# RViMLab/MICCAI2021_Cataract_semantic_segmentation

Hardware: AMD Instinct MI355X
Metric: train frames/sec @540x960 OCRNet-HRNetw48 (higher is better)
Workload: dtype f32 (convolutions with K >= 2048 and >= 192 output columns, and the 3x3 trunk convolutions of the HRNet widths: forward / backward-data of those with > 192 output columns: operands scaled by a per-tensor power of two and split into 2 fp16 planes (22 significant bits), 3 fp16 MFMA products; forward /

## Files before the change

### include/catseg_debug.h

```cpp
#ifndef CATSEG_DEBUG_H
#define CATSEG_DEBUG_H

#include "catseg.h"

#ifdef __cplusplus
extern "C" {
#endif

int catseg_debug_set_tile(int mi, int ni);
int catseg_debug_set_splits(int splits);
int catseg_debug_set_strided_multi(int on);
int catseg_debug_set_lovasz_prune(int on);
int catseg_debug_set_wgrad_direct(int on);

int catseg_debug_set_dconv3_blocks(int blocks);
int catseg_debug_set_dconv3_spec(int on);
int catseg_debug_set_dconv3_alt96(int on);
int catseg_debug_set_dwgrad3_blocks(int blocks);
int catseg_debug_set_dwgrad3_pl_blocks(int blocks);
int catseg_debug_set_dwgrad3_pl_form(int form);
int catseg_debug_set_dconv3_pl_slots(int slots);
int catseg_debug_set_dconv3_pl_pair(int mask);
int catseg_debug_dconv3_pl_occupancy(int C, int pair);
int catseg_debug_dwgrad3_pl_occupancy(int C);

int catseg_debug_set_h2w_slow_epilogue(int on);

int catseg_debug_set_b3_tile(int t);
int catseg_debug_plan_conv(const catseg_conv_desc* d, int op, int* out);

int catseg_debug_set_bilinear_bwd_fused(int on);
int catseg_debug_set_h2w_waves(int waves);

int catseg_debug_set_pconv1_wgrad_blocks(int n);

#ifdef __cplusplus
}
#endif
#endif
```

### miccai2021_cataract_semantic_segmentation_amd/_lib.py

```python
import ctypes as C
import os

import torch

_HERE = os.path.dirname(os.path.abspath(__file__))
LIB_PATH = os.environ.get("CATSEG_LIB") or os.path.join(_HERE, "libcatseg_hip.so")

if not os.path.exists(LIB_PATH):
    raise ImportError(
        "libcatseg_hip.so is missing (%s). Build it with `python -c 'import __graft_entry__ as g; g.build()'` "
        "or `make -C miccai2021_cataract_semantic_segmentation_amd/csrc`. There is no CPU fallback." % LIB_PATH)

lib = C.CDLL(LIB_PATH)

P, I, L, F, SZ = C.c_void_p, C.c_int, C.c_longlong, C.c_float, C.c_size_t


class ConvDesc(C.Structure):
    _fields_ = [(n, I) for n in ("B", "H", "W", "Cin", "Ho", "Wo", "Cout", "kh", "kw", "stride", "pad", "dil",
                                 "ldx", "ldy", "stem4", "groups")]


class BnApplyDesc(C.Structure):
    _fields_ = [("y", P), ("ldy", I), ("mean", P), ("scale", P), ("beta", P), ("residual", P), ("ldr", I), ("residual_record", P), ("z", P), ("ldz", I),
# ... 36 lines not shown
    "catseg_dconv3_pl_rows": (I, [I, I, I, I]),
    "catseg_planes_bytes": (SZ, [L, I]),
    "catseg_planes_from_f32": (I, [P, I, L, I, P, P, I, P]),
    "catseg_dconv3_pl": (I, [I, I, I, I, P, P, P, P, P, P, I, I, P, SZ, P, P, P]),
    "catseg_dconv3_pl_bnbwd": (I, [I, I, I, I, P, P, P, P, P, I, P, I, P, P, P, P, SZ, P, P]),
    "catseg_dwgrad3_pl_supported": (I, [I]),
    "catseg_dwgrad3_pl_workspace": (SZ, [I, I, I, I]),
    "catseg_dwgrad3_pl": (I, [I, I, I, I, P, P, P, P, P, P, SZ, P]),
    "catseg_bn_finalize_counts_bound": (I, [P, I, P, L, I, P, P, F, F, P, P, P, P, P, P, P]),
    "catseg_bn_backward_h2_workspace": (SZ, [L, I]),
    "catseg_head_fwd": (I, [P, I, P, P, P, P, P, I, L, I, P, I, I, P]),
    "catseg_head_backward_workspace": (SZ, [L, I]),
    "catseg_head_backward": (I, [P, I, P, I, P, P, P, P, I, L, I, P, P, P, P, P, P, P, P, P, P, P, SZ, P]),
    "catseg_head_fwd_drop": (I, [P, I, P, P, P, P, P, I, L, I, P, I, I, P, L, F, P]),
    "catseg_head_backward_drop": (I, [P, I, P, I, P, P, P, P, I, L, I, P, P, P, P, P, P, P, P, P, P, P, SZ, P, L, F, P]),
    "catseg_dropout2d_mask": (I, [P, F, I, I, P, P, P]),
    "catseg_dropout2d_mask_fixed": (I, [P, F, I, I, P, P, P]),
    "catseg_dropout2d_apply": (I, [P, I, P, L, I, L, P, I, P]),
    "catseg_maxpool2x2_fwd": (I, [P, I, P, I, P, I, I, I, I, P]),
    "catseg_maxpool2x2_bwd": (I, [P, I, P, P, I, I, I, I, I, P]),
    "catseg_bias_rows": (I, [P, P, I, L, I, P]),
    "catseg_bn_mask_bytes": (SZ, [L, I]),
    "catseg_conv2d_fwd_fused": (I, [P, P, P, P, P, I, I, P, P]),
    "catseg_fold_bn": (I, [P, P, P, P, P, P, F, I, I, P, P, P]),
    "catseg_conv2d_bwd_data": (I, [P, P, P, P, I, P]),
    "catseg_conv2d_bwd_weight_workspace": (SZ, [P]),
    "catseg_conv2d_bwd_weight": (I, [P, P, P, P, P, P, SZ, P]),
    "catseg_gemm_batched": (I, [I, I, I, I, I, P, I, L, P, I, L, P, I, L, I, I, P]),
    "catseg_sum_slabs": (I, [P, P, L, I, I, I, P]),
    "catseg_debug_set_tile": (I, [I, I]),
    "catseg_debug_set_splits": (I, [I]),
    "catseg_debug_set_strided_multi": (I, [I]),
    "catseg_debug_set_lovasz_prune": (I, [I]),
    "catseg_debug_set_wgrad_direct": (I, [I]),
    "catseg_debug_plan_conv": (I, [P, I, P]),
    "catseg_debug_set_b3_tile": (I, [I]),
    "catseg_debug_set_dconv3_blocks": (I, [I]),
    "catseg_debug_set_dconv3_pl_slots": (I, [I]),
    "catseg_debug_set_dconv3_pl_pair": (I, [I]),
    "catseg_debug_set_dwgrad3_pl_blocks": (I, [I]),
    "catseg_debug_set_dwgrad3_pl_form": (I, [I]),
    "catseg_debug_dconv3_pl_occupancy": (I, [I, I]),
    "catseg_debug_dwgrad3_pl_occupancy": (I, [I]),
    "catseg_debug_set_dconv3_spec": (I, [I]),
    "catseg_debug_set_dconv3_alt96": (I, [I]),
    "catseg_aug_pad_flip_u8": (I, [P, P, I, I, I, I, P, I, I, P]),
    "catseg_aug_box_blur": (I, [P, P, I, I, I, I, P, P, P, P]),
    "catseg_aug_color_op": (I, [P, I, I, I, P, P, P, SZ, P]),
    "catseg_split3_elems": (SZ, [L, I]),
    "catseg_split3": (I, [P, I, L, I, P, P]),
    "catseg_split3_weight_t": (I, [P, I, I, I, P, P]),
    "catseg_split3_blocked_elems": (SZ, [L, I]),
    "catseg_split3_blocked": (I, [P, L, I, I, P, P, P]),
    "catseg_split3_weight_blocked": (I, [P, I, I, I, P, P]),
    "catseg_split3_weight_t_blocked": (I, [P, I, I, I, P, P]),
    "catseg_conv2d_fwd_bf16x3_blocked": (I, [P, P, P, P, P, I, P, SZ, P, P, P]),
    "catseg_conv2d_bwd_data_bf16x3_blocked": (I, [P, P, P, P, I, P]),
    "catseg_conv2d_fwd_fused_bf16x3_blocked": (I, [P, P, P, P, P, I, I, P, P]),
    "catseg_split2h_blocked_elems": (SZ, [L, I]),
    "catseg_split2h_planar_elems": (SZ, [L, I]),
    "catseg_split2h": (I, [P, L, I, I, P, P, P, P]),
    "catseg_split2h_bound": (I, [P, L, I, I, P, P, P, P, P, P, P, P]),
    "catseg_conv2d_bwd_weight_f16x2_workspace": (SZ, [P]),
    "catseg_conv2d_bwd_weight_f16x2": (I, [P, P, P, P, P, P, P, SZ, P]),
    "catseg_conv2d_bwd_weight_f16x2_blocked": (I, [P, P, P, P, P, P, P, SZ, P]),
    "catseg_concat_bilinear_split2h": (I, [I, P, P, P, P, P, P, I, I, I, P, P, P]),
# ... 133 lines not shown
```

### miccai2021_cataract_semantic_segmentation_amd/csrc/lovasz.hip

```cpp
#include "common.h"
#include "rows.h"

namespace {

constexpr int RBITS = 8;
constexpr int RADIX = 1 << RBITS;
constexpr int SORT_PASSES = 4;
constexpr int SORT_BLOCKS = 128;
constexpr int TILE = 4096;
constexpr int PIX = 256;
constexpr int MAXK = 64;

struct LvWs {
  uint32_t* counts;
  uint32_t* keys[2];
  uint32_t* vals[2];
  uint32_t* hist;
  uint32_t* fgsum;
  float* lpart;
  float* dprob;
  double* lossd;
  uint32_t* minfg;
  uint32_t* nact;
  uint32_t* blkcnt;
// ... 8 lines not shown
    return p;
  };
  const long long ntiles = (P + TILE - 1) / TILE;
  LvWs t;
  t.counts = (uint32_t*)take((MAXK + 4) * 4);
  for (int i = 0; i < 2; ++i) {
    t.keys[i] = (uint32_t*)take((size_t)K * P * 4);
    t.vals[i] = (uint32_t*)take((size_t)K * P * 4);
  }
  t.hist = (uint32_t*)take((size_t)K * RADIX * SORT_BLOCKS * 4);
  t.fgsum = (uint32_t*)take((size_t)K * ntiles * 4);
  t.lpart = (float*)take((size_t)K * ntiles * 4);
  t.dprob = (float*)take((size_t)K * P * 4);
  t.lossd = (double*)take(64);
  t.minfg = (uint32_t*)take(MAXK * 4);
  t.nact = (uint32_t*)take(MAXK * 4);
  t.blkcnt = (uint32_t*)take((size_t)K * ((P + PIX - 1) / PIX) * 4);
  t.actmask = (unsigned long long*)take((size_t)P * 8);
  if (w) *w = t;
  return off;
}

__global__ void label_hist_kernel(const int64_t* __restrict__ labels, long long P, int K, uint32_t* __restrict__ counts) {
  __shared__ uint32_t h[MAXK];
  if (threadIdx.x < MAXK) h[threadIdx.x] = 0;
  __syncthreads();
  for (long long i = blockIdx.x * (long long)blockDim.x + threadIdx.x; i < P; i += (long long)gridDim.x * blockDim.x) {
    const int64_t l = labels[i];
    if (l >= 0 && l < K) atomicAdd(&h[(int)l], 1u);
  }
  __syncthreads();
  if (threadIdx.x < K && h[threadIdx.x]) atomicAdd(&counts[threadIdx.x], h[threadIdx.x]);
}
__global__ void present_kernel(int K, uint32_t* counts) {
  if (threadIdx.x == 0) {
    uint32_t n = 0;
    for (int c = 0; c < K; ++c) n += counts[c] != 0;
    counts[MAXK] = n;
  }
}

__global__ __launch_bounds__(PIX) void lv_prep_kernel(const float* __restrict__ logits, const int64_t* __restrict__ labels, long long P,
                                                      int K, const uint32_t* __restrict__ counts, uint32_t* __restrict__ keys,
                                                      uint32_t* __restrict__ vals) {
  extern __shared__ float sh[];
  const int KS = K | 1;
  const long long p0 = (long long)blockIdx.x * PIX;
  const int np = (int)min((long long)PIX, P - p0);
  stage_rows(logits, p0, np, K, KS, sh);
  __syncthreads();
  const int t = threadIdx.x;
  if (t >= np) return;
  float* row = sh + t * KS;
  float m = row[0];
  for (int c = 1; c < K; ++c) m = fmaxf(m, row[c]);
  float s = 0.f;
  for (int c = 0; c < K; ++c) {
    const float e = expf(row[c] - m);
    row[c] = e;
    s += e;
  }
  const long long p = p0 + t;
  const int64_t lab = labels[p];
  for (int c = 0; c < K; ++c) {
    if (counts[c] == 0) continue;
    const float pr = row[c] / s;
    const uint32_t fg = (lab == c) ? 1u : 0u;
    const float err = fabsf((float)fg - pr);
    keys[(long long)c * P + p] = 0x3F800000u - __float_as_uint(err);
    vals[(long long)c * P + p] = (uint32_t)p | (fg << 31);
  }
}

__device__ __forceinline__ void softmax_row(float* row, int K, float& s) {
  float m = row[0];
  for (int c = 1; c < K; ++c) m = fmaxf(m, row[c]);
  s = 0.f;
  for (int c = 0; c < K; ++c) {
    const float e = expf(row[c] - m);
    row[c] = e;
    s += e;
  }
}

__global__ __launch_bounds__(PIX) void lv_minfg_kernel(const float* __restrict__ logits, const int64_t* __restrict__ labels, long long P, int K,
                                                       uint32_t* __restrict__ minfg) {
  extern __shared__ float sh[];
  __shared__ uint32_t mn[MAXK];
  const int KS = K | 1;
  const long long p0 = (long long)blockIdx.x * PIX;
  const int np = (int)min((long long)PIX, P - p0);
  if (threadIdx.x < MAXK) mn[threadIdx.x] = 0x7F7F7F7Fu;
  stage_rows(logits, p0, np, K, KS, sh);
  __syncthreads();
  const int t = threadIdx.x;
  if (t < np) {
    const int64_t lab = labels[p0 + t];
    if (lab >= 0 && lab < K) {
      float* row = sh + t * KS;
      float s;
      softmax_row(row, K, s);
      const float err = fabsf(1.f - row[(int)lab] / s);
      atomicMin(&mn[(int)lab], __float_as_uint(err));
    }
  }
  __syncthreads();
  if (threadIdx.x < K && mn[threadIdx.x] != 0x7F7F7F7Fu) atomicMin(&minfg[threadIdx.x], mn[threadIdx.x]);
}

__global__ __launch_bounds__(PIX) void lv_compact1_kernel(const float* __restrict__ logits, const int64_t* __restrict__ labels, long long P, int K,
                                                          const uint32_t* __restrict__ counts, const uint32_t* __restrict__ minfg,
                                                          uint32_t* __restrict__ blkcnt, long long nblk, uint32_t* __restrict__ tmp,
                                                          unsigned long long* __restrict__ actmask) {
  extern __shared__ float sh[];
  __shared__ uint32_t wcnt[4][MAXK];
  const int KS = K | 1;
  const long long p0 = (long long)blockIdx.x * PIX;
  const int np = (int)min((long long)PIX, P - p0);
  stage_rows(logits, p0, np, K, KS, sh);
  __syncthreads();
  const int t = threadIdx.x, lane = t & 63, wave = t >> 6;
  const bool live = t < np;
  float* row = sh + t * KS;
  float s = 1.f;
  int64_t lab = -1;
  if (live) {
    softmax_row(row, K, s);
    lab = labels[p0 + t];
  }
  const unsigned long long lt_mask = (lane == 0) ? 0ull : (~0ull >> (64 - lane));
  unsigned long long bits = 0;
  for (int c = 0; c < K; ++c) {
    bool a = false;
    if (live && counts[c] != 0) {
      const uint32_t fg = (lab == c) ? 1u : 0u;
      const float err = fabsf((float)fg - row[c] / s);
      a = fg || __float_as_uint(err) >= minfg[c];
      if (a) row[c] = err;
    }
    const unsigned long long bal = __ballot(a);
// ... 329 lines not shown
      if (dp) dp[vv[j] & 0x7FFFFFFFu] = (err == 0.f) ? 0.f : (f ? -g : g);
    }
  }
  loss = wave_sum(loss);
  if (lane == 0) lsum[wave] = loss;
  __syncthreads();
  if (tid == 0) lpart[(long long)c * ntiles + blockIdx.x] = lsum[0] + lsum[1] + lsum[2] + lsum[3];
}

__global__ __launch_bounds__(256) void lv_finalize_kernel(const uint32_t* __restrict__ counts, const float* __restrict__ lpart, long long ntiles,
                                                          int K, float weight, float* __restrict__ loss_out, int accumulate) {
  __shared__ double sh[256];
  double tot = 0;
  for (int c = 0; c < K; ++c) {
    if (counts[c] == 0) continue;
    double s0 = 0, s1 = 0, s2 = 0, s3 = 0;
    long long i = threadIdx.x;
    for (; i + 768 < ntiles; i += 1024) {
      s0 += lpart[(long long)c * ntiles + i];
      s1 += lpart[(long long)c * ntiles + i + 256];
      s2 += lpart[(long long)c * ntiles + i + 512];
      s3 += lpart[(long long)c * ntiles + i + 768];
    }
    for (; i < ntiles; i += 256) s0 += lpart[(long long)c * ntiles + i];
    tot += (s0 + s1) + (s2 + s3);
  }
  sh[threadIdx.x] = tot;
  __syncthreads();
  for (int o = 128; o > 0; o >>= 1) {
    if (threadIdx.x < o) sh[threadIdx.x] += sh[threadIdx.x + o];
    __syncthreads();
  }
  if (threadIdx.x == 0) {
    const uint32_t n = counts[MAXK];
    const float l = n ? (float)(sh[0] / (double)n) * weight : 0.f;
    loss_out[0] = accumulate ? loss_out[0] + l : l;
  }
}

__global__ __launch_bounds__(PIX) void lv_backward_kernel(const float* __restrict__ logits, long long P, int K, const uint32_t* __restrict__ counts,
                                                          const float* __restrict__ dprob, float weight, float* __restrict__ dlogits, int acc,
                                                          const float* __restrict__ upstream, const unsigned long long* __restrict__ actmask,
                                                          const uint32_t* __restrict__ blkoff, long long nblk) {
  extern __shared__ float sh[];
  __shared__ uint32_t wcnt[4][MAXK];
  const int KS = K | 1;
  const long long p0 = (long long)blockIdx.x * PIX;
  const int np = (int)min((long long)PIX, P - p0);
  stage_rows(logits, p0, np, K, KS, sh);
  const int t = threadIdx.x;
  unsigned long long bits = 0;
  if (actmask) {
    const int lane = t & 63, wave = t >> 6;
    if (t < np) bits = actmask[p0 + t];
    for (int c = 0; c < K; ++c) {
      const unsigned long long bal = __ballot((bits >> c) & 1ull);
      if (lane == 0) wcnt[wave][c] = (uint32_t)__popcll(bal);
    }
    __syncthreads();
    if (t < K) {
      const uint32_t b = blkoff[(long long)t * nblk + blockIdx.x], w0 = wcnt[0][t], w1 = wcnt[1][t], w2 = wcnt[2][t];
      wcnt[0][t] = b; wcnt[1][t] = b + w0; wcnt[2][t] = b + w0 + w1; wcnt[3][t] = b + w0 + w1 + w2;
    }
  }
  __syncthreads();
  if (t < np) {
    float* row = sh + t * KS;
    float m = row[0];
    for (int c = 1; c < K; ++c) m = fmaxf(m, row[c]);
    float s = 0.f;
    for (int c = 0; c < K; ++c) {
      const float e = expf(row[c] - m);
      row[c] = e;
      s += e;
    }
    const uint32_t npres = counts[MAXK];
    const float w = npres ? weight / (float)npres : 0.f;
    const long long p = p0 + t;
    float* grow = sh + PIX * KS + t * KS;
    float dot = 0.f;
    for (int c0 = 0; c0 < K; c0 += 8) {
      float gv[8];
      if (actmask) {
        const int lane = t & 63, wave = t >> 6;
        const unsigned long long lt_mask = (lane == 0) ? 0ull : (~0ull >> (64 - lane));
#pragma unroll
        for (int u = 0; u < 8; ++u) {
          const int c = c0 + u;
          gv[u] = 0.f;
          if (c < K) {
            const bool a = (bits >> c) & 1ull;
            const unsigned long long bal = __ballot(a);
            if (a) gv[u] = dprob[(long long)c * P + wcnt[wave][c] + (uint32_t)__popcll(bal & lt_mask)];
          }
        }
      } else {
#pragma unroll
        for (int u = 0; u < 8; ++u) {
          const int c = c0 + u;
          gv[u] = (c < K && counts[c]) ? dprob[(long long)c * P + p] : 0.f;
        }
      }
#pragma unroll
      for (int u = 0; u < 8; ++u) {
        const int c = c0 + u;
        if (c < K) {
          const float pr = row[c] / s;
          const float g = gv[u] * w;
          row[c] = pr;
          grow[c] = g;
          dot += g * pr;
        }
      }
    }
    const float up = upstream ? *upstream : 1.f;
    for (int c = 0; c < K; ++c) {
      const float v = row[c] * (grow[c] - dot);
      row[c] = upstream ? v * up : v;
    }
  }
  __syncthreads();
  unstage_rows(dlogits, p0, np, K, KS, sh, acc != 0);
}

__global__ __launch_bounds__(PIX) void ce_fwd_kernel(const float* __restrict__ logits, const int64_t* __restrict__ labels, long long P, int K,
                                                     long long ignore, float* __restrict__ part) {
  extern __shared__ float sh[];
  const int KS = K | 1;
  const long long p0 = (long long)blockIdx.x * PIX;
  const int np = (int)min((long long)PIX, P - p0);
  stage_rows(logits, p0, np, K, KS, sh);
  __syncthreads();
  const int t = threadIdx.x;
  float l = 0.f, cnt = 0.f;
  if (t < np) {
    const int64_t lab = labels[p0 + t];
    if (lab != ignore && lab >= 0 && lab < K) {
      const float* row = sh + t * KS;
      float m = row[0];
      for (int c = 1; c < K; ++c) m = fmaxf(m, row[c]);
      float s = 0.f;
      for (int c = 0; c < K; ++c) s += expf(row[c] - m);
      l = logf(s) + m - row[(int)lab];
      cnt = 1.f;
    }
  }
  l = wave_sum(l);
  cnt = wave_sum(cnt);
  __shared__ float r[8];
  if ((t & 63) == 0) { r[t >> 6] = l; r[4 + (t >> 6)] = cnt; }
  __syncthreads();
  if (t == 0) {
    part[2 * blockIdx.x] = r[0] + r[1] + r[2] + r[3];
    part[2 * blockIdx.x + 1] = r[4] + r[5] + r[6] + r[7];
  }
// ... 65 lines not shown
  __syncthreads();
  for (int i = threadIdx.x; i < K * K; i += blockDim.x)
    if (hist[i]) atomicAdd(&cm[i], hist[i]);
}

__global__ void adam_kernel(float* __restrict__ p, const float* __restrict__ g, float* __restrict__ m, float* __restrict__ v, long long n4,
                            long long n, float lr, float b1, float b2, float eps, float bc1, float bc2s, float gscale,
                            const float* __restrict__ hyper) {
  if (hyper) {
    lr = hyper[0]; bc1 = hyper[1]; bc2s = hyper[2]; gscale = hyper[3];
  }
  for (long long i = blockIdx.x * (long long)blockDim.x + threadIdx.x; i < n4; i += (long long)gridDim.x * blockDim.x) {
    const long long e = i * 4;
    if (e + 3 < n) {
      f32x4 gg = *(const f32x4*)(g + e) * gscale;
      f32x4 mm = *(f32x4*)(m + e) * b1 + gg * (1.f - b1);
      f32x4 vv = *(f32x4*)(v + e) * b2 + gg * gg * (1.f - b2);
      f32x4 pp = *(f32x4*)(p + e);
#pragma unroll
      for (int k = 0; k < 4; ++k) pp[k] -= (lr / bc1) * (mm[k] / (sqrtf(vv[k]) / bc2s + eps));
      *(f32x4*)(m + e) = mm; *(f32x4*)(v + e) = vv; *(f32x4*)(p + e) = pp;
    } else {
      for (long long j = e; j < n; ++j) {
        const float gg = g[j] * gscale;
        const float mm = m[j] * b1 + gg * (1.f - b1);
        const float vv = v[j] * b2 + gg * gg * (1.f - b2);
        m[j] = mm; v[j] = vv;
        p[j] -= (lr / bc1) * (mm / (sqrtf(vv) / bc2s + eps));
      }
    }
  }
}

int g_prune = 1;

}

extern "C" int catseg_debug_set_lovasz_prune(int on) {
  g_prune = on ? 1 : 0;
  return CATSEG_OK;
}

extern "C" size_t catseg_lovasz_workspace(long long P, int K) { return lv_layout(P, K, nullptr, nullptr); }

namespace {
int lovasz_run(const float* logits, const int64_t* labels, long long P, int K, float weight, float* loss_out, float* dlogits, int want_grad,
               int accumulate_dlogits, void* workspace, size_t workspace_bytes, catseg_stream_t stream) {
  CS_REQUIRE(P > 0 && P < (1ll << 31) && K > 0 && K <= MAXK, "lovasz: need 0 < P < 2^31 and K <= %d", MAXK);
  const size_t need = lv_layout(P, K, nullptr, nullptr);
  if (workspace_bytes < need || !workspace) {
    catseg_set_error("lovasz: workspace %zu < %zu", workspace_bytes, need);
    return CATSEG_EWORKSPACE;
  }
  hipStream_t st = (hipStream_t)stream;
  LvWs w;
  lv_layout(P, K, (char*)workspace, &w);
  const long long ntiles = (P + TILE - 1) / TILE;
  const int nb = (int)((P + PIX - 1) / PIX);
  const size_t shb = (size_t)PIX * (K | 1) * 4;
  if (g_prune) {
    CS_LDS_RESERVE(lv_minfg_kernel, shb, "lovasz");
    CS_LDS_RESERVE(lv_compact1_kernel, shb, "lovasz");
  } else {
    CS_LDS_RESERVE(lv_prep_kernel, shb, "lovasz");
  }
  if (dlogits) CS_LDS_RESERVE(lv_backward_kernel, 2 * shb, "lovasz backward");
  if (hipMemsetAsync(w.counts, 0, (MAXK + 4) * 4, st) != hipSuccess) { catseg_set_error("lovasz: memset failed"); return CATSEG_EHIP; }
  hipLaunchKernelGGL(label_hist_kernel, dim3(nb < 1024 ? nb : 1024), dim3(256), 0, st, labels, P, K, w.counts);
  hipLaunchKernelGGL(present_kernel, dim3(1), dim3(64), 0, st, K, w.counts);
  if (g_prune) {
    if (hipMemsetAsync(w.minfg, 0x7F, MAXK * 4, st) != hipSuccess) { catseg_set_error("lovasz: memset failed"); return CATSEG_EHIP; }
    hipLaunchKernelGGL(lv_minfg_kernel, dim3(nb), dim3(PIX), shb, st, logits, labels, P, K, w.minfg);
    hipLaunchKernelGGL(lv_compact1_kernel, dim3(nb), dim3(PIX), shb, st, logits, labels, P, K, (const uint32_t*)w.counts,
                       (const uint32_t*)w.minfg, w.blkcnt, (long long)nb, w.keys[1], w.actmask);
    hipLaunchKernelGGL(lv_blkscan_kernel, dim3(K), dim3(1024), 0, st, (const uint32_t*)w.counts, w.blkcnt, (long long)nb, w.nact);
    hipLaunchKernelGGL(lv_gather_kernel, dim3(nb), dim3(PIX), 0, st, (const uint32_t*)w.keys[1], P, K, (const uint32_t*)w.counts,
                       (const uint32_t*)w.blkcnt, (long long)nb, (const uint32_t*)w.nact, w.keys[0], w.vals[0]);
  } else {
    hipLaunchKernelGGL(lv_fill_nact_kernel, dim3(1), dim3(64), 0, st, w.nact, (uint32_t)P);
    hipLaunchKernelGGL(lv_prep_kernel, dim3(nb), dim3(PIX), shb, st, logits, labels, P, K, (const uint32_t*)w.counts, w.keys[0], w.vals[0]);
  }
  const uint32_t* nact = (const uint32_t*)w.nact;
  int cur = 0;
  for (int pass = 0; pass < SORT_PASSES; ++pass) {
    const int shift = pass * RBITS;
    hipLaunchKernelGGL(radix_upsweep_kernel, dim3(SORT_BLOCKS, K), dim3(256), 0, st, (const uint32_t*)w.keys[cur], P, shift, (const uint32_t*)w.counts, nact, w.hist);
    hipLaunchKernelGGL(radix_scan_kernel, dim3(K), dim3(1024), 0, st, (const uint32_t*)w.counts, w.hist);
    hipLaunchKernelGGL(radix_downsweep_kernel, dim3(SORT_BLOCKS, K), dim3(256), 0, st, (const uint32_t*)w.keys[cur], (const uint32_t*)w.vals[cur],
                       w.keys[cur ^ 1], w.vals[cur ^ 1], P, shift, (const uint32_t*)w.counts, nact, (const uint32_t*)w.hist);
    cur ^= 1;
  }
  hipLaunchKernelGGL(lv_fgsum_kernel, dim3((unsigned)ntiles, K), dim3(256), 0, st, (const uint32_t*)w.vals[cur], P, (const uint32_t*)w.counts, nact, w.fgsum, ntiles);
  hipLaunchKernelGGL(lv_fgscan_kernel, dim3(K), dim3(1024), 0, st, (const uint32_t*)w.counts, w.fgsum, ntiles);
  hipLaunchKernelGGL(lv_grad_kernel, dim3((unsigned)ntiles, K), dim3(256), 0, st, (const uint32_t*)w.keys[cur], (const uint32_t*)w.vals[cur], P,
                     (const uint32_t*)w.counts, nact, (const uint32_t*)w.fgsum, ntiles, w.lpart, want_grad ? w.dprob : nullptr);
  hipLaunchKernelGGL(lv_finalize_kernel, dim3(1), dim3(256), 0, st, (const uint32_t*)w.counts, (const float*)w.lpart, ntiles, K, weight, loss_out, 0);
  if (dlogits)
    hipLaunchKernelGGL(lv_backward_kernel, dim3(nb), dim3(PIX), 2 * shb, st, logits, P, K, (const uint32_t*)w.counts, (const float*)w.dprob, weight, dlogits,
                       accumulate_dlogits, (const float*)nullptr, g_prune ? (const unsigned long long*)w.actmask : nullptr, (const uint32_t*)w.blkcnt,
                       (long long)nb);
  CS_LAUNCH_CHECK();
  return CATSEG_OK;
}
}

extern "C" int catseg_lovasz_softmax(const float* logits, const int64_t* labels, long long P, int K, float weight,
                                     float* loss_out, float* dlogits, int accumulate_dlogits, void* workspace,
                                     size_t workspace_bytes, catseg_stream_t stream) {
  return lovasz_run(logits, labels, P, K, weight, loss_out, dlogits, dlogits != nullptr, accumulate_dlogits, workspace, workspace_bytes, stream);
}

extern "C" int catseg_lovasz_softmax_fwd(const float* logits, const int64_t* labels, long long P, int K, float weight, float* loss_out,
                                         int want_grad, void* workspace, size_t workspace_bytes, catseg_stream_t stream) {
  return lovasz_run(logits, labels, P, K, weight, loss_out, nullptr, want_grad, 0, workspace, workspace_bytes, stream);
}

extern "C" int catseg_lovasz_softmax_bwd(const float* logits, long long P, int K, float weight, const float* upstream, float* dlogits,
                                         int accumulate_dlogits, void* workspace, size_t workspace_bytes, catseg_stream_t stream) {
  CS_REQUIRE(P > 0 && P < (1ll << 31) && K > 0 && K <= MAXK && logits && dlogits && workspace, "lovasz bwd: bad args");
  CS_REQUIRE(workspace_bytes >= lv_layout(P, K, nullptr, nullptr), "lovasz bwd: workspace too small");
  LvWs w;
  lv_layout(P, K, (char*)workspace, &w);
  const int nb = (int)((P + PIX - 1) / PIX);
  const size_t shb = (size_t)PIX * (K | 1) * 4;
  CS_LDS_RESERVE(lv_backward_kernel, 2 * shb, "lovasz backward");
  hipLaunchKernelGGL(lv_backward_kernel, dim3(nb), dim3(PIX), 2 * shb, (hipStream_t)stream, logits, P, K, (const uint32_t*)w.counts, (const float*)w.dprob, weight,
                     dlogits, accumulate_dlogits, upstream, g_prune ? (const unsigned long long*)w.actmask : nullptr, (const uint32_t*)w.blkcnt, (long long)nb);
  CS_LAUNCH_CHECK();
  return CATSEG_OK;
}

extern "C" size_t catseg_ce_workspace(long long P) { return cs_align_up((size_t)((P + PIX - 1) / PIX) * 8 + 256, 256); }

extern "C" int catseg_cross_entropy(const float* logits, const int64_t* labels, long long P, int K, long long ignore_index,
                                    float weight, float* loss_out, float* dlogits, void* workspace,
                                    size_t workspace_bytes, catseg_stream_t stream) {
  CS_REQUIRE(P > 0 && K > 0 && K <= MAXK, "ce: bad args");
  if (workspace_bytes < catseg_ce_workspace(P) || !workspace) {
    catseg_set_error("ce: workspace too small");
    return CATSEG_EWORKSPACE;
  }
  hipStream_t st = (hipStream_t)stream;
  const int nb = (int)((P + PIX - 1) / PIX);
  const size_t shb = (size_t)PIX * (K | 1) * 4;
  float* inv = (float*)workspace;
  float* part = inv + 64;
  CS_LDS_RESERVE(ce_fwd_kernel, shb, "ce");
  if (dlogits) CS_LDS_RESERVE(ce_bwd_kernel, shb, "ce backward");
  hipLaunchKernelGGL(ce_fwd_kernel, dim3(nb), dim3(PIX), shb, st, logits, labels, P, K, ignore_index, part);
  hipLaunchKernelGGL(ce_finalize_kernel, dim3(1), dim3(256), 0, st, (const float*)part, (long long)nb, weight, loss_out, inv);
  if (dlogits) hipLaunchKernelGGL(ce_bwd_kernel, dim3(nb), dim3(PIX), shb, st, logits, labels, P, K, ignore_index, weight, (const float*)inv, dlogits);
  CS_LAUNCH_CHECK();
  return CATSEG_OK;
}

extern "C" int catseg_confusion_matrix(const float* logits, const int64_t* labels, long long P, int K, int32_t* cm,
                                       catseg_stream_t stream) {
  CS_REQUIRE(P > 0 && K > 0 && K <= MAXK, "confusion: bad args");
  const int nb = (int)((P + PIX - 1) / PIX);
  const size_t shb = (size_t)PIX * (K | 1) * 4 + (size_t)K * K * 4;
// ... 43 lines not shown
```

Before: 81.65.

## Make Lovasz minfg and backward passes persistent with double-buffered tile prefetch

Both per-pixel Lovasz passes, minfg and backward, now launch a resident grid sized from the occupancy query. Each block loops over tiles and fetches the next tile's logits into registers while the current tile is processed from a double-buffered LDS area. The label histogram is folded into the minfg pass, and the memsets plus present-count kernel are replaced by one small arm kernel. This cuts launch and serialization overhead and hides load latency, at the cost of more registers and more complex indexing in a loss step that is a small part of the training iteration.

```diff
diff --git a/include/catseg_debug.h b/include/catseg_debug.h
--- a/include/catseg_debug.h
+++ b/include/catseg_debug.h
@@ -11,6 +11,7 @@
 int catseg_debug_set_splits(int splits);
 int catseg_debug_set_strided_multi(int on);
 int catseg_debug_set_lovasz_prune(int on);
+int catseg_debug_lovasz_pass_grid(int pass, int K);
 int catseg_debug_set_wgrad_direct(int on);
 
 int catseg_debug_set_dconv3_blocks(int blocks);
diff --git a/miccai2021_cataract_semantic_segmentation_amd/_lib.py b/miccai2021_cataract_semantic_segmentation_amd/_lib.py
--- a/miccai2021_cataract_semantic_segmentation_amd/_lib.py
+++ b/miccai2021_cataract_semantic_segmentation_amd/_lib.py
@@ -92,6 +92,7 @@
     "catseg_debug_set_splits": (I, [I]),
     "catseg_debug_set_strided_multi": (I, [I]),
     "catseg_debug_set_lovasz_prune": (I, [I]),
+    "catseg_debug_lovasz_pass_grid": (I, [I, I]),
     "catseg_debug_set_wgrad_direct": (I, [I]),
     "catseg_debug_plan_conv": (I, [P, I, P]),
     "catseg_debug_set_b3_tile": (I, [I]),
diff --git a/miccai2021_cataract_semantic_segmentation_amd/csrc/lovasz.hip b/miccai2021_cataract_semantic_segmentation_amd/csrc/lovasz.hip
--- a/miccai2021_cataract_semantic_segmentation_amd/csrc/lovasz.hip
+++ b/miccai2021_cataract_semantic_segmentation_amd/csrc/lovasz.hip
@@ -64,11 +64,10 @@
   __syncthreads();
   if (threadIdx.x < K && h[threadIdx.x]) atomicAdd(&counts[threadIdx.x], h[threadIdx.x]);
 }
-__global__ void present_kernel(int K, uint32_t* counts) {
-  if (threadIdx.x == 0) {
-    uint32_t n = 0;
-    for (int c = 0; c < K; ++c) n += counts[c] != 0;
-    counts[MAXK] = n;
+__global__ void lv_arm_kernel(uint32_t* __restrict__ counts, uint32_t* __restrict__ minfg) {
+  if (threadIdx.x < MAXK) {
+    counts[threadIdx.x] = 0;
+    minfg[threadIdx.x] = 0x7F7F7F7Fu;
   }
 }
 
@@ -115,29 +114,132 @@
   }
 }
 
-__global__ __launch_bounds__(PIX) void lv_minfg_kernel(const float* __restrict__ logits, const int64_t* __restrict__ labels, long long P, int K,
-                                                       uint32_t* __restrict__ minfg) {
-  extern __shared__ float sh[];
-  __shared__ uint32_t mn[MAXK];
-  const int KS = K | 1;
-  const long long p0 = (long long)blockIdx.x * PIX;
-  const int np = (int)min((long long)PIX, P - p0);
-  if (threadIdx.x < MAXK) mn[threadIdx.x] = 0x7F7F7F7Fu;
-  stage_rows(logits, p0, np, K, KS, sh);
-  __syncthreads();
-  const int t = threadIdx.x;
-  if (t < np) {
-    const int64_t lab = labels[p0 + t];
+extern __shared__ __attribute__((aligned(16))) uint32_t lvsh[];
+constexpr size_t LV_SCRATCH[2] = {2 * MAXK * 4, (8 * MAXK + 4) * 4};
+template <int KB> struct TileRegs { float4 q[2 * KB]; float tail; };
+constexpr int lv_waves(int KB) { return KB <= 2 ? 4 : KB <= 4 ? 3 : 1; }
+
+template <int KB>
+__device__ __forceinline__ void tile_fetch(const float* __restrict__ logits, long long p0, int np, int K, TileRegs<KB>& r) {
+  const int n = np * K, tid = threadIdx.x;
+  const float* src = logits + p0 * K;
+  const int mis = (int)((reinterpret_cast<uintptr_t>(src) >> 2) & 3);
+  const float4* s4 = reinterpret_cast<const float4*>(src - mis);
+  const int nq = min((n + mis + 3) >> 2, 2 * KB * PIX);
+#pragma unroll
+  for (int u = 0; u < 2 * KB; ++u) r.q[u] = s4[min(u * PIX + tid, nq - 1)];
+  const int cov = 4 * nq - mis;
+  if (cov < n) {
+    const int i = cov + tid;
+    if (i < n) r.tail = src[i];
+  }
+}
+template <int KB>
+__device__ __forceinline__ void tile_commit(const float* __restrict__ logits, const TileRegs<KB>& r, long long p0, int np, int K, int KS, float* sh) {
+  const int n = np * K, tid = threadIdx.x;
+  const int mis = (int)((reinterpret_cast<uintptr_t>(logits + p0 * K) >> 2) & 3);
+  const int nq = min((n + mis + 3) >> 2, 2 * KB * PIX), cov = 4 * nq - mis;
+  int Kq = K;
+  asm volatile("" : "+s"(Kq));
+  if (mis == 0 && KS == K) {
+    float4* d4 = reinterpret_cast<float4*>(sh);
+#pragma unroll
+    for (int u = 0; u < 2 * KB; ++u) {
+      const int i4 = u * PIX + tid;
+      if (i4 < nq) d4[i4] = r.q[u];
+    }
+  } else if (mis == 0) {
+#pragma unroll
+    for (int u = 0; u < 2 * KB; ++u) {
+      const int i4 = u * PIX + tid;
+      if (i4 < nq) {
+        const float e[4] = {r.q[u].x, r.q[u].y, r.q[u].z, r.q[u].w};
+        int rr = (4 * i4) / Kq, c = 4 * i4 - rr * Kq;
+#pragma unroll
+        for (int q = 0; q < 4; ++q) {
+          if (4 * i4 + q < n) sh[rr * KS + c] = e[q];
+          if (++c == Kq) { c = 0; ++rr; }
+        }
+      }
+    }
+  } else {
+#pragma unroll
+    for (int u = 0; u < 2 * KB; ++u) {
+      const int i4 = u * PIX + tid;
+      if (i4 < nq) {
+        const float e[4] = {r.q[u].x, r.q[u].y, r.q[u].z, r.q[u].w};
+#pragma unroll
+        for (int q = 0; q < 4; ++q) {
+          const int i = 4 * i4 - mis + q;
+          if (i >= 0 && i < n) { const int rr = i / Kq; sh[rr * KS + (i - rr * Kq)] = e[q]; }
+        }
+      }
+    }
+  }
+  if (cov < n) {
+    const int i = cov + tid;
+    if (i < n) { const int rr = i / Kq; sh[rr * KS + (i - rr * Kq)] = r.tail; }
+  }
+}
+__device__ __forceinline__ void tile_unstage(float* __restrict__ out, long long p0, int np, int K, int KS, const float* sh, bool acc) {
+  float* dst = out + p0 * K;
+  if (KS != K || (reinterpret_cast<uintptr_t>(dst) & 15) != 0) { unstage_rows(out, p0, np, K, KS, sh, acc); return; }
+  const int n = np * K, n4 = n >> 2;
+  float4* d4 = reinterpret_cast<float4*>(dst);
+  const float4* s4 = reinterpret_cast<const float4*>(sh);
+  for (int i4 = threadIdx.x; i4 < n4; i4 += PIX) {
+    float4 v = s4[i4];
+    if (acc) {
+      const float4 o = d4[i4];
+      v.x += o.x; v.y += o.y; v.z += o.z; v.w += o.w;
+    }
+    d4[i4] = v;
+  }
+  for (int i = (n4 << 2) + threadIdx.x; i < n; i += PIX) dst[i] = acc ? dst[i] + sh[i] : sh[i];
+}
+__device__ __forceinline__ int tile_pixels(long long tile, long long P) { return (int)min((long long)PIX, P - tile * PIX); }
+
+template <int KB>
+__global__ __launch_bounds__(PIX, lv_waves(KB)) void lv_minfg_kernel(const float* __restrict__ logits, const int64_t* __restrict__ labels, long long P, int K,
+                                                       long long ntile, uint32_t* __restrict__ minfg, uint32_t* __restrict__ counts) {
+  uint32_t* mn = lvsh;
+  uint32_t* hc = lvsh + MAXK;
+  float* rows = reinterpret_cast<float*>(lvsh + 2 * MAXK);
+  const int KS = K | 1, t = threadIdx.x;
+  if (t < MAXK) { mn[t] = 0x7F7F7F7Fu; hc[t] = 0; }
+  long long tile = blockIdx.x;
+  TileRegs<KB> r;
+  int64_t labn = -1;
+  if (tile < ntile) {
+    const int np = tile_pixels(tile, P);
+    tile_fetch(logits, tile * PIX, np, K, r);
+    if (t < np) labn = labels[tile * PIX + t];
+    tile_commit(logits, r, tile * PIX, np, K, KS, rows);
+  }
+  __syncthreads();
+  for (int cur = 0; tile < ntile; tile += gridDim.x, cur ^= 1) {
+    const long long nxt = tile + gridDim.x;
+    const int64_t lab = labn;
+    const long long pre = nxt < ntile ? nxt : tile;
+    const int npn = tile_pixels(pre, P);
+    tile_fetch(logits, pre * PIX, npn, K, r);
+    labn = labels[min(pre * PIX + t, P - 1)];
+    if (t >= npn) labn = -1;
     if (lab >= 0 && lab < K) {
-      float* row = sh + t * KS;
+      float* row = rows + cur * PIX * KS + t * KS;
       float s;
       softmax_row(row, K, s);
       const float err = fabsf(1.f - row[(int)lab] / s);
       atomicMin(&mn[(int)lab], __float_as_uint(err));
-    }
-  }
-  __syncthreads();
-  if (threadIdx.x < K && mn[threadIdx.x] != 0x7F7F7F7Fu) atomicMin(&minfg[threadIdx.x], mn[threadIdx.x]);
+      atomicAdd(&hc[(int)lab], 1u);
+    }
+    if (nxt < ntile) tile_commit(logits, r, nxt * PIX, npn, K, KS, rows + (cur ^ 1) * PIX * KS);
+    __syncthreads();
+  }
+  if (t < K && hc[t]) {
+    atomicAdd(&counts[t], hc[t]);
+    atomicMin(&minfg[t], mn[t]);
+  }
 }
 
 __global__ __launch_bounds__(PIX) void lv_compact1_kernel(const float* __restrict__ logits, const int64_t* __restrict__ labels, long long P, int K,
@@ -533,95 +635,125 @@
     __syncthreads();
   }
   if (threadIdx.x == 0) {
-    const uint32_t n = counts[MAXK];
+    uint32_t n = 0;
+    for (int c = 0; c < K; ++c) n += counts[c] != 0;
     const float l = n ? (float)(sh[0] / (double)n) * weight : 0.f;
     loss_out[0] = accumulate ? loss_out[0] + l : l;
   }
 }
 
-__global__ __launch_bounds__(PIX) void lv_backward_kernel(const float* __restrict__ logits, long long P, int K, const uint32_t* __restrict__ counts,
-                                                          const float* __restrict__ dprob, float weight, float* __restrict__ dlogits, int acc,
-                                                          const float* __restrict__ upstream, const unsigned long long* __restrict__ actmask,
-                                                          const uint32_t* __restrict__ blkoff, long long nblk) {
-  extern __shared__ float sh[];
-  __shared__ uint32_t wcnt[4][MAXK];
+template <int KB, bool PRUNED>
+__global__ __launch_bounds__(PIX, lv_waves(KB)) void lv_backward_kernel(const float* __restrict__ logits, long long P, int K, long long ntile,
+                                                          const uint32_t* __restrict__ counts, const float* __restrict__ dprob, float weight,
+                                                          float* __restrict__ dlogits, int acc, const float* __restrict__ upstream,
+                                                          const unsigned long long* __restrict__ actmask, const uint32_t* __restrict__ blkoff) {
+  uint32_t (*wcnt)[4][MAXK] = reinterpret_cast<uint32_t (*)[4][MAXK]>(lvsh);
+  uint32_t& snpres = lvsh[8 * MAXK];
+  float* rows = reinterpret_cast<float*>(lvsh + 8 * MAXK + 4);
   const int KS = K | 1;
-  const long long p0 = (long long)blockIdx.x * PIX;
-  const int np = (int)min((long long)PIX, P - p0);
-  stage_rows(logits, p0, np, K, KS, sh);
-  const int t = threadIdx.x;
-  unsigned long long bits = 0;
-  if (actmask) {
-    const int lane = t & 63, wave = t >> 6;
-    if (t < np) bits = actmask[p0 + t];
-    for (int c = 0; c < K; ++c) {
-      const unsigned long long bal = __ballot((bits >> c) & 1ull);
-      if (lane == 0) wcnt[wave][c] = (uint32_t)__popcll(bal);
-    }
-    __syncthreads();
-    if (t < K) {
-      const uint32_t b = blkoff[(long long)t * nblk + blockIdx.x], w0 = wcnt[0][t], w1 = wcnt[1][t], w2 = wcnt[2][t];
-      wcnt[0][t] = b; wcnt[1][t] = b + w0; wcnt[2][t] = b + w0 + w1; wcnt[3][t] = b + w0 + w1 + w2;
-    }
-  }
-  __syncthreads();
-  if (t < np) {
-    float* row = sh + t * KS;
-    float m = row[0];
-    for (int c = 1; c < K; ++c) m = fmaxf(m, row[c]);
-    float s = 0.f;
-    for (int c = 0; c < K; ++c) {
-      const float e = expf(row[c] - m);
-      row[c] = e;
-      s += e;
-    }
-    const uint32_t npres = counts[MAXK];
-    const float w = npres ? weight / (float)npres : 0.f;
-    const long long p = p0 + t;
-    float* grow = sh + PIX * KS + t * KS;
-    float dot = 0.f;
-    for (int c0 = 0; c0 < K; c0 += 8) {
-      float gv[8];
-      if (actmask) {
-        const int lane = t & 63, wave = t >> 6;
-        const unsigned long long lt_mask = (lane == 0) ? 0ull : (~0ull >> (64 - lane));
-#pragma unroll
-        for (int u = 0; u < 8; ++u) {
-          const int c = c0 + u;
-          gv[u] = 0.f;
-          if (c < K) {
-            const bool a = (bits >> c) & 1ull;
-            const unsigned long long bal = __ballot(a);
-            if (a) gv[u] = dprob[(long long)c * P + wcnt[wave][c] + (uint32_t)__popcll(bal & lt_mask)];
-          }
-        }
+  const int t = threadIdx.x, lane = t & 63, wave = t >> 6;
+  const unsigned long long lt_mask = (lane == 0) ? 0ull : (~0ull >> (64 - lane));
+  if (wave == 0) {
+    const unsigned long long pres = __ballot(t < K && counts[t] != 0);
+    if (lane == 0) snpres = (uint32_t)__popcll(pres);
+  }
+  long long tile = blockIdx.x;
+  TileRegs<KB> r;
+  unsigned long long bitsn = 0;
+  uint32_t boffn = 0;
+  if (tile < ntile) {
+    const int np = tile_pixels(tile, P);
+    tile_fetch(logits, tile * PIX, np, K, r);
+    if (PRUNED) {
+      if (t < np) bitsn = actmask[tile * PIX + t];
+      if (t < K) boffn = blkoff[(long long)t * ntile + tile];
+      for (int c = 0; c < K; ++c) {
+        const unsigned long long bal = __ballot((bitsn >> c) & 1ull);
+        if (lane == 0) wcnt[0][wave][c] = (uint32_t)__popcll(bal);
+      }
+    }
+    tile_commit(logits, r, tile * PIX, np, K, KS, rows);
+  }
+  __syncthreads();
+  if (PRUNED && tile < ntile && t < K) {
+    const uint32_t b = boffn, w0 = wcnt[0][0][t], w1 = wcnt[0][1][t], w2 = wcnt[0][2][t];
+    wcnt[0][0][t] = b; wcnt[0][1][t] = b + w0; wcnt[0][2][t] = b + w0 + w1; wcnt[0][3][t] = b + w0 + w1 + w2;
+  }
+  __syncthreads();
+  const uint32_t npres = snpres;
+  const float w = npres ? weight / (float)npres : 0.f;
+  const float up = upstream ? *upstream : 1.f;
+  for (int cur = 0; tile < ntile; tile += gridDim.x, cur ^= 1) {
+    const long long nxt = tile + gridDim.x, p0 = tile * PIX;
+    const int np = tile_pixels(tile, P);
+    const unsigned long long bits = bitsn;
+    float gv[8 * KB];
+#pragma unroll
+    for (int c = 0; c < 8 * KB; ++c) {
+      const int cc = min(c, K - 1);
+      if (PRUNED) {
+        const bool a = (bits >> c) & 1ull;
+        const unsigned long long bal = __ballot(a);
+        gv[c] = dprob[(long long)cc * P + (a ? wcnt[cur][wave][cc] + (uint32_t)__popcll(bal & lt_mask) : 0u)];
       } else {
-#pragma unroll
-        for (int u = 0; u < 8; ++u) {
-          const int c = c0 + u;
-          gv[u] = (c < K && counts[c]) ? dprob[(long long)c * P + p] : 0.f;
-        }
-      }
-#pragma unroll
-      for (int u = 0; u < 8; ++u) {
-        const int c = c0 + u;
+        gv[c] = dprob[(long long)cc * P + min(p0 + t, P - 1)];
+      }
+    }
+    const long long pre = nxt < ntile ? nxt : tile;
+    const int npn = tile_pixels(pre, P);
+    tile_fetch(logits, pre * PIX, npn, K, r);
+    if (PRUNED) {
+      bitsn = actmask[min(pre * PIX + t, P - 1)];
+      if (t >= npn) bitsn = 0ull;
+      boffn = blkoff[(long long)min(t, K - 1) * ntile + pre];
+    }
+    float* buf = rows + cur * PIX * KS;
+    if (t < np) {
+      float* row = buf + t * KS;
+      float m = row[0];
+      for (int c = 1; c < K; ++c) m = fmaxf(m, row[c]);
+      float s = 0.f;
+      for (int c = 0; c < K; ++c) {
+        const float e = expf(row[c] - m);
+        row[c] = e;
+        s += e;
+      }
+      float dot = 0.f;
+#pragma unroll
+      for (int c = 0; c < 8 * KB; ++c) {
         if (c < K) {
           const float pr = row[c] / s;
-          const float g = gv[u] * w;
+          const float g = ((PRUNED ? (bits >> c) & 1ull : counts[c] != 0) ? gv[c] : 0.f) * w;
           row[c] = pr;
-          grow[c] = g;
+          gv[c] = g;
           dot += g * pr;
         }
       }
-    }
-    const float up = upstream ? *upstream : 1.f;
-    for (int c = 0; c < K; ++c) {
-      const float v = row[c] * (grow[c] - dot);
-      row[c] = upstream ? v * up : v;
-    }
-  }
-  __syncthreads();
-  unstage_rows(dlogits, p0, np, K, KS, sh, acc != 0);
+#pragma unroll
+      for (int c = 0; c < 8 * KB; ++c) {
+        if (c < K) {
+          const float v = row[c] * (gv[c] - dot);
+          row[c] = upstream ? v * up : v;
+        }
+      }
+    }
+    if (PRUNED && nxt < ntile) {
+      for (int c = 0; c < K; ++c) {
+        const unsigned long long bal = __ballot((bitsn >> c) & 1ull);
+        if (lane == 0) wcnt[cur ^ 1][wave][c] = (uint32_t)__popcll(bal);
+      }
+    }
+    __syncthreads();
+    if (nxt < ntile) {
+      tile_commit(logits, r, nxt * PIX, npn, K, KS, rows + (cur ^ 1) * PIX * KS);
+      if (PRUNED && t < K) {
+        const uint32_t b = boffn, w0 = wcnt[cur ^ 1][0][t], w1 = wcnt[cur ^ 1][1][t], w2 = wcnt[cur ^ 1][2][t];
+        wcnt[cur ^ 1][0][t] = b; wcnt[cur ^ 1][1][t] = b + w0; wcnt[cur ^ 1][2][t] = b + w0 + w1; wcnt[cur ^ 1][3][t] = b + w0 + w1 + w2;
+      }
+    }
+    tile_unstage(dlogits, p0, np, K, KS, buf, acc != 0);
+    __syncthreads();
+  }
 }
 
 __global__ __launch_bounds__(PIX) void ce_fwd_kernel(const float* __restrict__ logits, const int64_t* __restrict__ labels, long long P, int K,
@@ -753,13 +885,80 @@
   }
 }
 
+enum { LV_MINFG = 0, LV_BACKWARD = 1 };
+#define LV_KB_SWITCH(K, ...)                                                                   \
+  switch (((K) + 7) / 8) {                                                                     \
+    case 1: { constexpr int KB = 1; __VA_ARGS__; } break;  case 2: { constexpr int KB = 2; __VA_ARGS__; } break; \
+    case 3: { constexpr int KB = 3; __VA_ARGS__; } break;  case 4: { constexpr int KB = 4; __VA_ARGS__; } break; \
+    case 5: { constexpr int KB = 5; __VA_ARGS__; } break;  case 6: { constexpr int KB = 6; __VA_ARGS__; } break; \
+    case 7: { constexpr int KB = 7; __VA_ARGS__; } break;  default: { constexpr int KB = 8; __VA_ARGS__; } break; \
+  }
+size_t lv_pass_lds(int pass, int K) { return LV_SCRATCH[pass] + 2 * (size_t)PIX * (K | 1) * 4; }
+
+template <class Kernel>
+int lv_resident_grid(Kernel* kernel, size_t dyn, int* grid) {
+  int dev = 0, cus = 0, occ = 0;
+  if (hipGetDevice(&dev) != hipSuccess || hipDeviceGetAttribute(&cus, hipDeviceAttributeMultiprocessorCount, dev) != hipSuccess ||
+      hipOccupancyMaxActiveBlocksPerMultiprocessor(&occ, kernel, PIX, dyn) != hipSuccess || cus <= 0 || occ <= 0) {
+    (void)hipGetLastError();
+    catseg_set_error("lovasz: cannot size the grid of a per-pixel pass (%d CUs x %d blocks)", cus, occ);
+    return CATSEG_EHIP;
+  }
+  *grid = cus * occ;
+  return CATSEG_OK;
+}
+int lv_pass_grid(int pass, int K, int* grid) {
+  static int cache[2][MAXK + 1];
+  const size_t dyn = lv_pass_lds(pass, K);
+  int rc = CATSEG_OK;
+  LV_KB_SWITCH(K, {
+    if (pass == LV_MINFG) { rc = cs_lds_reserve(lv_minfg_kernel<KB>, dyn, "lovasz"); if (rc == CATSEG_OK && !cache[pass][K]) rc = lv_resident_grid(lv_minfg_kernel<KB>, dyn, &cache[pass][K]); }
+    else {
+      rc = cs_lds_reserve(lv_backward_kernel<KB, true>, dyn, "lovasz backward");
+      if (rc == CATSEG_OK) rc = cs_lds_reserve(lv_backward_kernel<KB, false>, dyn, "lovasz backward");
+      if (rc == CATSEG_OK && !cache[pass][K]) rc = lv_resident_grid(lv_backward_kernel<KB, true>, dyn, &cache[pass][K]);
+    }
+  });
+  if (rc == CATSEG_OK) *grid = cache[pass][K];
+  return rc;
+}
+#define LV_PASS_GRID(pass, K, grid)                      \
+  do {                                                   \
+    const int rc__ = lv_pass_grid(pass, K, &(grid));     \
+    if (rc__ != CATSEG_OK) return rc__;                  \
+  } while (0)
+
 int g_prune = 1;
+
+int lv_backward_launch(const float* logits, long long P, int K, const LvWs& w, float weight, float* dlogits, int acc, const float* upstream,
+                       hipStream_t st) {
+  const int nb = (int)((P + PIX - 1) / PIX);
+  int grid = 0;
+  LV_PASS_GRID(LV_BACKWARD, K, grid);
+  if (grid > nb) grid = nb;
+  const size_t lds = lv_pass_lds(LV_BACKWARD, K);
+  LV_KB_SWITCH(K, {
+    if (g_prune)
+      hipLaunchKernelGGL((lv_backward_kernel<KB, true>), dim3(grid), dim3(PIX), lds, st, logits, P, K, (long long)nb, (const uint32_t*)w.counts,
+                         (const float*)w.dprob, weight, dlogits, acc, upstream, (const unsigned long long*)w.actmask, (const uint32_t*)w.blkcnt);
+    else
+      hipLaunchKernelGGL((lv_backward_kernel<KB, false>), dim3(grid), dim3(PIX), lds, st, logits, P, K, (long long)nb, (const uint32_t*)w.counts,
+                         (const float*)w.dprob, weight, dlogits, acc, upstream, (const unsigned long long*)nullptr, (const uint32_t*)nullptr);
+  });
+  return CATSEG_OK;
+}
 
 }
 
 extern "C" int catseg_debug_set_lovasz_prune(int on) {
   g_prune = on ? 1 : 0;
   return CATSEG_OK;
+}
+
+extern "C" int catseg_debug_lovasz_pass_grid(int pass, int K) {
+  int g = -1;
+  if (pass < 0 || pass > 1 || K <= 0 || K > MAXK || lv_pass_grid(pass, K, &g) != CATSEG_OK) return -1;
+  return g;
 }
 
 extern "C" size_t catseg_lovasz_workspace(long long P, int K) { return lv_layout(P, K, nullptr, nullptr); }
@@ -779,25 +978,25 @@
   const long long ntiles = (P + TILE - 1) / TILE;
   const int nb = (int)((P + PIX - 1) / PIX);
   const size_t shb = (size_t)PIX * (K | 1) * 4;
+  int g_minfg = 0, g_bwd = 0;
   if (g_prune) {
-    CS_LDS_RESERVE(lv_minfg_kernel, shb, "lovasz");
+    LV_PASS_GRID(LV_MINFG, K, g_minfg);
     CS_LDS_RESERVE(lv_compact1_kernel, shb, "lovasz");
   } else {
     CS_LDS_RESERVE(lv_prep_kernel, shb, "lovasz");
   }
-  if (dlogits) CS_LDS_RESERVE(lv_backward_kernel, 2 * shb, "lovasz backward");
-  if (hipMemsetAsync(w.counts, 0, (MAXK + 4) * 4, st) != hipSuccess) { catseg_set_error("lovasz: memset failed"); return CATSEG_EHIP; }
-  hipLaunchKernelGGL(label_hist_kernel, dim3(nb < 1024 ? nb : 1024), dim3(256), 0, st, labels, P, K, w.counts);
-  hipLaunchKernelGGL(present_kernel, dim3(1), dim3(64), 0, st, K, w.counts);
+  if (dlogits) LV_PASS_GRID(LV_BACKWARD, K, g_bwd);
+  hipLaunchKernelGGL(lv_arm_kernel, dim3(1), dim3(MAXK), 0, st, w.counts, w.minfg);
   if (g_prune) {
-    if (hipMemsetAsync(w.minfg, 0x7F, MAXK * 4, st) != hipSuccess) { catseg_set_error("lovasz: memset failed"); return CATSEG_EHIP; }
-    hipLaunchKernelGGL(lv_minfg_kernel, dim3(nb), dim3(PIX), shb, st, logits, labels, P, K, w.minfg);
+    LV_KB_SWITCH(K, hipLaunchKernelGGL(lv_minfg_kernel<KB>, dim3(g_minfg < nb ? g_minfg : nb), dim3(PIX), lv_pass_lds(LV_MINFG, K), st, logits, labels, P, K,
+                                       (long long)nb, w.minfg, w.counts));
     hipLaunchKernelGGL(lv_compact1_kernel, dim3(nb), dim3(PIX), shb, st, logits, labels, P, K, (const uint32_t*)w.counts,
                        (const uint32_t*)w.minfg, w.blkcnt, (long long)nb, w.keys[1], w.actmask);
     hipLaunchKernelGGL(lv_blkscan_kernel, dim3(K), dim3(1024), 0, st, (const uint32_t*)w.counts, w.blkcnt, (long long)nb, w.nact);
     hipLaunchKernelGGL(lv_gather_kernel, dim3(nb), dim3(PIX), 0, st, (const uint32_t*)w.keys[1], P, K, (const uint32_t*)w.counts,
                        (const uint32_t*)w.blkcnt, (long long)nb, (const uint32_t*)w.nact, w.keys[0], w.vals[0]);
   } else {
+    hipLaunchKernelGGL(label_hist_kernel, dim3(nb < 1024 ? nb : 1024), dim3(256), 0, st, labels, P, K, w.counts);
     hipLaunchKernelGGL(lv_fill_nact_kernel, dim3(1), dim3(64), 0, st, w.nact, (uint32_t)P);
     hipLaunchKernelGGL(lv_prep_kernel, dim3(nb), dim3(PIX), shb, st, logits, labels, P, K, (const uint32_t*)w.counts, w.keys[0], w.vals[0]);
   }
@@ -816,10 +1015,10 @@
   hipLaunchKernelGGL(lv_grad_kernel, dim3((unsigned)ntiles, K), dim3(256), 0, st, (const uint32_t*)w.keys[cur], (const uint32_t*)w.vals[cur], P,
                      (const uint32_t*)w.counts, nact, (const uint32_t*)w.fgsum, ntiles, w.lpart, want_grad ? w.dprob : nullptr);
   hipLaunchKernelGGL(lv_finalize_kernel, dim3(1), dim3(256), 0, st, (const uint32_t*)w.counts, (const float*)w.lpart, ntiles, K, weight, loss_out, 0);
-  if (dlogits)
-    hipLaunchKernelGGL(lv_backward_kernel, dim3(nb), dim3(PIX), 2 * shb, st, logits, P, K, (const uint32_t*)w.counts, (const float*)w.dprob, weight, dlogits,
-                       accumulate_dlogits, (const float*)nullptr, g_prune ? (const unsigned long long*)w.actmask : nullptr, (const uint32_t*)w.blkcnt,
-                       (long long)nb);
+  if (dlogits) {
+    const int rc = lv_backward_launch(logits, P, K, w, weight, dlogits, accumulate_dlogits, nullptr, st);
+    if (rc != CATSEG_OK) return rc;
+  }
   CS_LAUNCH_CHECK();
   return CATSEG_OK;
 }
@@ -842,11 +1041,8 @@
   CS_REQUIRE(workspace_bytes >= lv_layout(P, K, nullptr, nullptr), "lovasz bwd: workspace too small");
   LvWs w;
   lv_layout(P, K, (char*)workspace, &w);
-  const int nb = (int)((P + PIX - 1) / PIX);
-  const size_t shb = (size_t)PIX * (K | 1) * 4;
-  CS_LDS_RESERVE(lv_backward_kernel, 2 * shb, "lovasz backward");
-  hipLaunchKernelGGL(lv_backward_kernel, dim3(nb), dim3(PIX), 2 * shb, (hipStream_t)stream, logits, P, K, (const uint32_t*)w.counts, (const float*)w.dprob, weight,
-                     dlogits, accumulate_dlogits, upstream, g_prune ? (const unsigned long long*)w.actmask : nullptr, (const uint32_t*)w.blkcnt, (long long)nb);
+  const int rc = lv_backward_launch(logits, P, K, w, weight, dlogits, accumulate_dlogits, upstream, (hipStream_t)stream);
+  if (rc != CATSEG_OK) return rc;
   CS_LAUNCH_CHECK();
   return CATSEG_OK;
 }
```

After: 81.91, median of 6. About the same (+0.3%).
